# flysoaryun/LF-VIO

Measured on AMD Instinct MI355X. Metric: sliding-window solves/sec (10 KF x N landmarks), higher is better.
Workload: dtype f64; 1 GPU; window300; landmarks=300, observations=1419, windows_per_gpu=1, marginalization=MARGIN_OLD, parallelism=1 independent window stream(s), one per GPU, no data-path collective

## Files before the change

lf-vio_amd/csrc/kernels_marg.h:

```cpp
#pragma once
#include "kernels_solve.h"

constexpr int MARG_THREADS = 768;
constexpr int MARG_MAXD = 96;
constexpr int LDN = 80;
constexpr double JACOBI_TOL = 1e-19;
constexpr size_t MARG_LDS = (size_t)19072 * sizeof(double);
constexpr int BT_GROUP = 4;

DEV void gauge_landmarks(Slot *S, int l0) {
  const int l = l0 + (int)threadIdx.x;
  double *lam = S->lam[S->tr.cur];
  if (l < S->N) lam[l] = 1.0 / (1.0 / lam[l]);
}
template <class T>
DEV void copy_rounds(T *dst, const T *src, int n, int tid, int nthr) {
  for (int k0 = tid; k0 < n; k0 += 8 * nthr) {
    T v[8];
#pragma unroll
    for (int q = 0; q < 8; q++) v[q] = src[k0 + q * nthr < n ? k0 + q * nthr : 0];
#pragma unroll
    for (int q = 0; q < 8; q++)
      if (k0 + q * nthr < n) dst[k0 + q * nthr] = v[q];
  }
}
DEV void gauge_poses(Slot *S, int gated, bool publish);
DEV void publish_solution(Slot *S) {
  char *m = (char *)S->mail;
  if (!m) return;
  const int tid = threadIdx.x, nthr = blockDim.x;
  const TRState *ts = &S->tr;
  const int cur = ts->cur, N = S->N;
  {
    constexpr int XW = (int)(sizeof(FrameState) / 8), XT = (XW + 63) / 64, LT = (SPEC_MAX_LM + 63) / 64, TT = 8;
    const double *xs = (const double *)&S->x[cur];
    double *xd = (double *)(m + MAIL_X + (size_t)cur * sizeof(FrameState));
    const long long *tsrc = (const long long *)ts;
    long long *tdst = (long long *)(m + MAIL_TR);
    const int tl = ts->trace_len < LFVIO_MAX_TRACE ? ts->trace_len : LFVIO_MAX_TRACE;
    const int words = (int)((offsetof(TRState, trace) + (size_t)(tl > 0 ? tl : 0) * sizeof(LfvioIterationSummary)) / 8);
    const double *ls = S->lam[cur];
    double *ld = (double *)(m + MAIL_LAM + (size_t)cur * MAIL_LAM_STRIDE);
    if (nthr >= 64 && XW <= XT * nthr && N <= LT * nthr && words <= TT * nthr) {
      double xv[XT], lv[LT];
      long long tv[TT];
#pragma unroll
      for (int k = 0; k < XT; k++) xv[k] = xs[tid + nthr * k < XW ? tid + nthr * k : 0];
#pragma unroll
      for (int k = 0; k < LT; k++) lv[k] = ls[tid + nthr * k < N ? tid + nthr * k : 0];
#pragma unroll
      for (int k = 0; k < TT; k++) tv[k] = tsrc[tid + nthr * k < words ? tid + nthr * k : 0];
#pragma unroll
      for (int k = 0; k < XT; k++)
        if (tid + nthr * k < XW) xd[tid + nthr * k] = xv[k];
#pragma unroll
      for (int k = 0; k < TT; k++)
        if (tid + nthr * k < words) tdst[tid + nthr * k] = tv[k];
#pragma unroll
      for (int k = 0; k < LT; k++)
        if (tid + nthr * k < N) ld[tid + nthr * k] = lv[k];
    } else {
      for (int k = tid; k < XW; k += nthr) xd[k] = xs[k];
      for (int k = tid; k < words; k += nthr) tdst[k] = tsrc[k];
      for (int k = tid; k < N; k += nthr) ld[k] = ls[k];
    }
  }
  if (tid == 0) ((int *)m)[4] = S->passes_used, ((int *)m)[5] = S->chain_err;
  __threadfence_system();
  __syncthreads();
  if (tid == 0) __hip_atomic_store((int *)m, S->mail_seq, __ATOMIC_RELEASE, __HIP_MEMORY_SCOPE_SYSTEM);
}
DEV void publish_prior(Slot *S) {
  char *m = (char *)S->mail;
  if (!m) return;
  const int tid = threadIdx.x, nthr = blockDim.x;
  const LfvioPrior *src = &S->prior_out;
  LfvioPrior *dst = (LfvioPrior *)(m + MAIL_PRIOR);
  const int n = src->valid == 1 ? src->n : 0;
  copy_rounds((long long *)dst, (const long long *)src, (int)(offsetof(LfvioPrior, linearized_jacobians) / 8), tid, nthr);
  copy_rounds(dst->linearized_jacobians, src->linearized_jacobians, n * n, tid, nthr);
  copy_rounds(dst->linearized_residuals, src->linearized_residuals, n, tid, nthr);
  if (tid == 0) ((int *)m)[2] = S->passes_used, ((int *)m)[3] = S->tr.iteration;
  __threadfence_system();
  __syncthreads();
  if (tid == 0) __hip_atomic_store((int *)m + 1, S->mail_seq, __ATOMIC_RELEASE, __HIP_MEMORY_SCOPE_SYSTEM);
}
__global__ __launch_bounds__(256) void k_publish(char *base, size_t stride) {
  Slot *S = SLOT(base, stride);
  if (!(S->tr.done && (S->tail_state == 0 || S->tail_state == 3))) return;
  publish_solution(S);
}
__global__ __launch_bounds__(256) void k_prior_chain(char *base, size_t stride) {
  Slot *S = SLOT(base, stride);
  const LfvioPrior *src = &S->prior_out;
  const int tid = threadIdx.x, n = S->prior_n, nb = S->prior_nb;
  __shared__ int late;
  if (tid == 0) {
    late = 0;
    const long long t0 = wall_clock64();
    while (spec_peek(&S->tail_state) == 3) {
      if (wall_clock64() - t0 > 10 * SPEC_WAIT_TICKS) {
        late = 1;
        break;
      }
      __builtin_amdgcn_s_sleep(8);
    }
    spec_acquire();
  }
  __syncthreads();
  __shared__ int differs;
  if (tid == 0) differs = 0;
  __syncthreads();
  const bool head = !late && src->valid == 1 && src->n == n && src->num_blocks == nb;
  if (head && tid < nb && !(src->blocks[tid].kind == S->prior_kind[tid] && src->blocks[tid].frame == S->prior_frame[tid] && src->block_idx[tid] == S->prior_idx[tid]))
    differs = 1;
  for (int i = 256 + tid; head && i < nb; i += 256)
    if (!(src->blocks[i].kind == S->prior_kind[i] && src->blocks[i].frame == S->prior_frame[i] && src->block_idx[i] == S->prior_idx[i])) differs = 1;
  __syncthreads();
  const bool same = head && !differs;
  if (!same) {
    if (tid == 0) S->prior_valid = 0, S->chain_err = 1;
    return;
  }
  double *J = S->prior_J, *r = S->prior_r;
  copy_rounds(J, src->linearized_jacobians, n * n, tid, 256);
  copy_rounds(r, src->linearized_residuals, n, tid, 256);
  copy_rounds(&S->prior_x0[0][0], &src->block_x0[0][0], nb * 9, tid, 256);
}
__global__ __launch_bounds__(128) void k_gauge(char *base, size_t stride, int gated) {
  Slot *S = SLOT(base, stride);
  if (gated && !tail_gate(S, S->tr.done)) return;
  if (blockIdx.x > 0) {
    gauge_landmarks(S, (blockIdx.x - 1) * 128);
    return;
  }
  gauge_poses(S, gated, false);
  if (gated && S->spec_on && threadIdx.x == 0) spec_settle(S);
}
__global__ __launch_bounds__(128) void k_decide_gauge(char *base, size_t stride, int publish) {
  Slot *S = SLOT(base, stride);
  decide_body(S);
  __syncthreads();
  if (!tail_gate(S, S->tr.done)) return;
  const int spec = S->spec_on;
  if (spec) {
    if (threadIdx.x == 0) spec_closing(S);
    __syncthreads();
  }
  {
    constexpr int LT = (SPEC_MAX_LM + 127) / 128;
    double *lam = S->lam[S->tr.cur];
    const int N = S->N, tid = threadIdx.x;
    double lv[LT];
#pragma unroll
    for (int k = 0; k < LT; k++) lv[k] = lam[tid + 128 * k < N ? tid + 128 * k : 0];
#pragma unroll
    for (int k = 0; k < LT; k++)
      if (tid + 128 * k < N) lam[tid + 128 * k] = 1.0 / (1.0 / lv[k]);
    for (int l0 = 128 * LT; l0 < N; l0 += 128) gauge_landmarks(S, l0);
  }
  gauge_poses(S, 1, publish != 0);
  if (spec && threadIdx.x == 0) spec_settle(S);
}
DEV void gauge_poses(Slot *S, int gated, bool publish) {
  TRState *ts = &S->tr;
  const int tid = threadIdx.x;
  __shared__ double rot[9], P0[3], oP0[3];
  FrameState *x = &S->x[ts->cur];
  if (tid == 0) {
    const m33 Rs0 = q2R(q_from_pose(S->x0.pose[0]));
    const m33 R00 = q2R(q_from_pose(x->pose[0]));
    const double h0 = sqrt(Rs0.a[0] * Rs0.a[0] + Rs0.a[3] * Rs0.a[3]), h00 = sqrt(R00.a[0] * R00.a[0] + R00.a[3] * R00.a[3]);
    const double c0 = Rs0.a[0] / h0, s0 = Rs0.a[3] / h0, c00 = R00.a[0] / h00, s00 = R00.a[3] / h00;
    const double cyd = c0 * c00 + s0 * s00, syd = s0 * c00 - c0 * s00;
    m33 rd;
    rd.a[0] = cyd, rd.a[1] = -syd, rd.a[2] = 0;
    rd.a[3] = syd, rd.a[4] = cyd, rd.a[5] = 0;
    rd.a[6] = 0, rd.a[7] = 0, rd.a[8] = 1;
    const double sin1deg = 0.017452406437283512;
    if (h0 < sin1deg || h00 < sin1deg) rd = mm(Rs0, tr(R00));
    for (int k = 0; k < 9; k++) rot[k] = rd.a[k];
    for (int k = 0; k < 3; k++) P0[k] = x->pose[0][k], oP0[k] = S->x0.pose[0][k];
  }
  __syncthreads();
  const m33 rd = ldm(rot);
  d3 Psi = mk3(0, 0, 0), Vsi = Psi;
  q4 qn = q4{1, 0, 0, 0};
  if (tid < 11) {
    const m33 Rsi = mm(rd, q2R(qnormalized(q_from_pose(x->pose[tid]))));
    Psi = mul(rd, ld3(x->pose[tid]) - ld3(P0)) + ld3(oP0);
    Vsi = mul(rd, ld3(x->sb[tid]));
    qn = R2q(Rsi);
  } else if (tid == 11) {
    qn = R2q(q2R(q_from_pose(x->ex)));
  }
  __syncthreads();
  __shared__ double bt[84 + TAB_SCRATCH];
  if (tid < 11) {
    const double pn[7] = {Psi.x, Psi.y, Psi.z, qn.x, qn.y, qn.z, qn.w};
#pragma unroll
    for (int k = 0; k < 7; k++) x->pose[tid][k] = pn[k], bt[7 * tid + k] = pn[k];
    x->sb[tid][0] = Vsi.x, x->sb[tid][1] = Vsi.y, x->sb[tid][2] = Vsi.z;
  } else if (tid == 11) {
    x->ex[3] = qn.x, x->ex[4] = qn.y, x->ex[5] = qn.z, x->ex[6] = qn.w;
#pragma unroll
    for (int k = 0; k < 3; k++) bt[77 + k] = x->ex[k];
    bt[80] = qn.x, bt[81] = qn.y, bt[82] = qn.z, bt[83] = qn.w;
  }
  __syncthreads();
  if (publish) publish_solution(S);
  if (tid == 0) {
    if (!gated) ts->done = 0;
    ts->do_lin = 1;
    ts->do_schur = 1;
    ts->chol_fail = 0;
  }
  build_tab(bt, &S->tab[ts->cur], tid, bt + 84);
}

__global__ __launch_bounds__(64) void k_spec_wait(char *base) {
  Slot *S = (Slot *)base;
  if (threadIdx.x != 0) return;
  const long long t0 = wall_clock64();
  while (spec_peek(&S->tail_state) == 3 && wall_clock64() - t0 < 10 * SPEC_WAIT_TICKS) __builtin_amdgcn_s_sleep(8);
}
__global__ __launch_bounds__(128) void k_spec_begin(char *base, size_t back) {
  Slot *S = (Slot *)base;
  Slot *S0 = (Slot *)(base - back);
  const int tid = threadIdx.x;
  __shared__ int sh_word, sh_go;
  const long long t0 = wall_clock64();
  for (;;) {
    if (tid == 0) {
      int go = 0, w = 0;
      const int last = S->shadow.last_word;
      for (;;) {
        const int f = spec_peek(&S0->spec.fin);
        w = spec_peek(&S0->spec.word);
        if (w != 0) {
          const int st = spec_ep(f) == spec_ep(w) ? spec_fin_state(f) : FIN_OPEN;
          if (st != FIN_OPEN) break;
          if (w != last) {
            go = 1;
            break;
          }
        }
        if (wall_clock64() - t0 > SPEC_WAIT_TICKS) break;
        __builtin_amdgcn_s_sleep(8);
      }
      spec_acquire();
      sh_word = w, sh_go = go;
    }
    __syncthreads();
    int go = __builtin_amdgcn_readfirstlane(sh_go);
    const int w = __builtin_amdgcn_readfirstlane(sh_word);
    if (!go) {
      if (tid == 0) S->shadow.word = 0, S->tr.done = 0;
      return;
    }
    const int ep = spec_ep(w), a = spec_acc(w), cur = w & 1;
    if (S->shadow.hdr_ep != ep) {
      const long long *src = (const long long *)S0;
      long long *dst = (long long *)S;
      constexpr int W0 = (int)(offsetof(Slot, lm_start) / 8), W1 = (int)(offsetof(Slot, x) / 8);
      static_assert(offsetof(Slot, lm_start) % 8 == 0 && offsetof(Slot, x) % 8 == 0, "header words");
      for (int k = tid; k < W1; k += 128) dst[k] = src[k] - (k >= W0 ? (long long)back : 0ll);
      const double *is = &S0->imu_sqrt[0][0];
      double *id = &S->imu_sqrt[0][0];
      for (int k = tid; k < LFVIO_WINDOW_SIZE * 225; k += 128) id[k] = is[k];
    }
    __syncthreads();
    {
      constexpr int XW = (int)(sizeof(FrameState) / 8), TW = (int)(sizeof(TRHead) / 8), XT = (XW + 127) / 128, LT = (SPEC_MAX_LM + 127) / 128;
      static_assert(TW <= 128, "the trust-region header in one trip");
      const double *xs = (const double *)&S0->x[cur];
      double *xd = (double *)&S->x[0];
      const double *ls = S0->lam[cur];
      double *ld = S->lam[0];
      const int N = S0->N;
      const long long *ts = (const long long *)&S0->tr;
      long long *td = (long long *)&S->tr;
      double xv[XT], lv[LT];
#pragma unroll
      for (int k = 0; k < XT; k++) xv[k] = xs[tid + 128 * k < XW ? tid + 128 * k : 0];
#pragma unroll
      for (int k = 0; k < LT; k++) lv[k] = ls[tid + 128 * k < N ? tid + 128 * k : 0];
      const long long tv = ts[tid < TW ? tid : 0];
#pragma unroll
      for (int k = 0; k < XT; k++)
        if (tid + 128 * k < XW) xd[tid + 128 * k] = xv[k];
#pragma unroll
      for (int k = 0; k < LT; k++)
        if (tid + 128 * k < N) ld[tid + 128 * k] = 1.0 / (1.0 / lv[k]);
      if (tid < TW) td[tid] = tv;
      for (int k = tid + 128 * LT; k < N; k += 128) ld[k] = 1.0 / (1.0 / ls[k]);
    }
    __syncthreads();
    if (tid == 0) {
      const int f = spec_ld(&S0->spec.fin), w2 = spec_ld(&S0->spec.word);
      const bool open = spec_ep(f) != ep || spec_fin_state(f) == FIN_OPEN;
      sh_go = (w2 == w && open && spec_cas(&S0->spec.own[a], SPEC_FREE, SPEC_SIDE) == SPEC_FREE) ? 1 : 0;
      S->shadow.hdr_ep = ep;
      S->shadow.last_word = w;
    }
    __syncthreads();
    go = __builtin_amdgcn_readfirstlane(sh_go);
    if (!go) {
      __syncthreads();
      continue;
    }
    if (tid == 0) {
      S->shadow.word = w, S->shadow.ticket = S0->spec.ticket;
      S->spec_on = 0, S->dec_pending = 0, S->tail_state = 0, S->chain_err = 0;
      S->tr.cur = 0, S->tr.done = 1;
    }
    __syncthreads();
    break;
  }
  gauge_poses(S, 1, false);
}

DEV bool spd_inverse_wave(const double *Am, double *Xout, int m, int lane, double floor) {
  double a[15];
#pragma unroll
  for (int j = 0; j < 15; j++) a[j] = (lane < m && j < m) ? Am[lane * m + j] : (lane == j ? 1.0 : 0.0);
  bool ok = true;
  double dinv = 1.0;
#pragma unroll
  for (int j = 0; j < 15; j++) {
    const double d = readlane_f64(a[j], j);
    ok = ok && (d > 0.0);
    const double rs = fast_rsqrt(d);
    const double l = lane == j ? d * rs : a[j] * rs;
    a[j] = l;
    dinv = lane == j ? rs : dinv;
#pragma unroll
    for (int c = j + 1; c < 15; c++) a[c] = fma(-l, readlane_f64(l, c), a[c]);
  }
  double y[15];
#pragma unroll
  for (int i = 0; i < 15; i++) {
    double t = lane == i ? 1.0 : 0.0;
#pragma unroll
    for (int k = 0; k < i; k++) t = fma(-readlane_f64(a[k], i), y[k], t);
    y[i] = t * readlane_f64(dinv, i);
  }
  double fro = 0;
#pragma unroll
  for (int r = 0; r < 15; r++) {
    double x = 0;
#pragma unroll
    for (int i = r; i < 15; i++) x = fma(readlane_f64(y[i], r), y[i], x);
    if (lane < m && r < m) Xout[r * m + lane] = x, fro += x * x;
  }
  fro = wave_sum(fro);
  return ok && fro * floor * floor < 1.0;
}

DEV void rr_pair(int k, int step, int np, int n, int &p, int &q) {
  if (k == 0) {
    p = step, q = np - 1;
  } else {
    p = step + k;
    if (p >= np - 1) p -= np - 1;
    q = step - k;
    if (q < 0) q += np - 1;
  }
  if (q >= n) q = -1;
}

DEV void jacobi_angle(double app, double aqq, double apq, double &c, double &s) {
  c = 1.0, s = 0.0;
  if (apq != 0.0 && fabs(apq) > 1e-18 * (fabs(app) + fabs(aqq))) {
#if defined(JAC_TRIVIAL)
    c = 0.8, s = 0.6;
#elif defined(JAC_IEEE)
    const double theta = (aqq - app) / (2.0 * apq);
    const double t = (theta >= 0 ? 1.0 : -1.0) / (fabs(theta) + sqrt(theta * theta + 1.0));
    c = rsqrt(t * t + 1.0);
    s = t * c;
#else
    const double d = aqq - app, e = 2.0 * apq;
    const double h2 = fma(d, d, e * e);
    const double h = h2 * fast_rsqrt(h2);
    const double t = (d >= 0 ? e : -e) * fast_rcp(fabs(d) + h);
    c = fast_rsqrt(fma(t, t, 1.0));
    s = t * c;
#endif
  }
}

DEV int jacobi_small(double *Am, double *Vm, int n, int tid, int nthreads, double *buf, double2 *cs, double *scratch) {
  const int np = n + (n & 1), half = np / 2;
  double *Ac = buf, *An = buf + 256, *Vc = buf + 512, *Vn = buf + 768;
  const bool act = tid < np * np;
  const int u = act ? tid / np : 0, v = act ? tid % np : 0;
  const int ku = u >> 1, bu = u & 1, kv = v >> 1, bv = v & 1;
  auto idx0 = [&](int p) { return (p & 1) ? np - 1 - (p >> 1) : (p >> 1); };
  auto sigma = [&](int p) {
    const int k = p >> 1;
    if (!(p & 1)) return k >= 1 ? 2 * (k - 1) : 3;
    if (k == 0) return 1;
    return k <= half - 2 ? 2 * (k + 1) + 1 : 2 * (half - 1);
  };
  if (act) {
    const int iu = idx0(u), iv = idx0(v);
    Ac[tid] = (iu < n && iv < n) ? Am[iu * n + iv] : 0.0;
    Vc[tid] = (u == iv) ? 1.0 : 0.0;
  }
  const int dst_a = sigma(u) * np + sigma(v), dst_v = u * np + sigma(v);
  const int blk = (2 * ku) * np + 2 * kv;
  __syncthreads();
  int sweeps = 0, g = 0;
  double prev_off = 1e300;
  for (int sweep = 0; sweep < JMAX_SWEEPS; sweep++) {
    double off = 0, dia = 0;
    if (act) {
      const double a = Ac[tid];
      if (u == v) dia = a * a;
      else off = a * a;
    }
    off = wave_sum(off), dia = wave_sum(dia);
    if ((tid & 63) == 0) scratch[tid >> 6] = off, scratch[16 + (tid >> 6)] = dia;
    __syncthreads();
    double so = 0, sd = 0;
    for (int w = 0; w < nthreads / 64; w++) so += scratch[w], sd += scratch[16 + w];
    __syncthreads();
    if (so <= 1e-24 * sd || so == 0.0) break;
    if (sweep >= 4 && so > 0.25 * prev_off) break;
    prev_off = so;
    sweeps++;
    for (int step = 0; step < np - 1; step++, g++) {
      if (tid < half) {
        const int p = 2 * tid, q = p + 1;
        double c = 1.0, s = 0.0;
        if (tid > 0 || np == n) jacobi_angle(Ac[p * np + p], Ac[q * np + q], Ac[q * np + p], c, s);
        cs[tid] = make_double2(c, s);
      }
      __syncthreads();
      if (act) {
        const double2 ra = cs[ku], rb = cs[kv];
        const double ru0 = bu ? ra.y : ra.x, ru1 = bu ? ra.x : -ra.y;
        const double cv0 = bv ? rb.y : rb.x, cv1 = bv ? rb.x : -rb.y;
        const double a00 = Ac[blk], a01 = Ac[blk + 1], a10 = Ac[blk + np], a11 = Ac[blk + np + 1];
        An[dst_a] = ru0 * fma(a00, cv0, a01 * cv1) + ru1 * fma(a10, cv0, a11 * cv1);
        Vn[dst_v] = fma(Vc[u * np + 2 * kv], cv0, Vc[u * np + 2 * kv + 1] * cv1);
      }
      __syncthreads();
      double *t = Ac;
      Ac = An, An = t, t = Vc, Vc = Vn, Vn = t;
    }
  }
  if (act) {
    int p, q;
    rr_pair(kv, g % (np - 1), np, n, p, q);
    const int iv = bv ? q : p;
    if (u == v && iv >= 0) Am[iv * n + iv] = Ac[tid];
    if (u < n && iv >= 0) Vm[u * n + iv] = Vc[tid];
  }
  __syncthreads();
  return sweeps;
}

typedef const __attribute__((address_space(4))) double sdouble;
#define STURM_TOUCH8(v) asm volatile("" ::"s"(v[0]), "s"(v[1]), "s"(v[2]), "s"(v[3]), "s"(v[4]), "s"(v[5]), "s"(v[6]), "s"(v[7]))
DEV int sturm_count(sdouble *Tg , int n, double sigma) {
  double pm = 1.0, p = Tg[0] - sigma;
  unsigned cnt = (unsigned)__double2hiint(p) >> 31;
  unsigned bits = (unsigned)__double2hiint(p) >> 31;
  double d0[8], e0[8], d1[8], e1[8];
#pragma unroll
  for (int u = 0; u < 8; u++) d0[u] = Tg[1 + u], e0[u] = Tg[96 + u];
  for (int i0 = 1; i0 < n; i0 += 16) {
    STURM_TOUCH8(d0);
    STURM_TOUCH8(e0);
#pragma unroll
    for (int u = 0; u < 8; u++) d1[u] = Tg[i0 + 8 + u], e1[u] = Tg[96 + i0 + 8 + u - 1];
#pragma unroll
    for (int u = 0; u < 8; u++) {
      const double pn = fma(d0[u] - sigma, p, -e0[u] * pm);
      bits = __builtin_amdgcn_alignbit(bits, (unsigned)__double2hiint(pn), 31);
      pm = p, p = pn;
    }
    STURM_TOUCH8(d1);
    STURM_TOUCH8(e1);
#pragma unroll
    for (int u = 0; u < 8; u++) d0[u] = Tg[i0 + 16 + u], e0[u] = Tg[96 + i0 + 16 + u - 1];
#pragma unroll
    for (int u = 0; u < 8; u++) {
      const double pn = fma(d1[u] - sigma, p, -e1[u] * pm);
      bits = __builtin_amdgcn_alignbit(bits, (unsigned)__double2hiint(pn), 31);
      pm = p, p = pn;
    }
    cnt += __builtin_popcount((bits ^ (bits >> 1)) & 0xffffu);
    const int ex = ilogb(fmax(fmax(fabs(p), fabs(pm)), 1e-300));
    p = ldexp(p, -ex), pm = ldexp(pm, -ex);
  }
  return (int)cnt;
}
struct TriCtx {
  double *dd, *ee, *tau, *vb0, *vb1, *pp, *RV;
  int n, r0, c0;
};
template <int P>
DEV void tri_finish_row(const TriCtx &tc, int kk, const double (&row)[5], bool own) {
  const int n = tc.n, c0 = tc.c0;
  double *vb = (kk & 1) ? tc.vb1 : tc.vb0;
  double a_part = 0.0, ss_part = 0.0, dk = 0.0;
  bool has_d = false;
#pragma unroll
  for (int q = P; q < 5; q++) {
    const int C = c0 + 16 * q;
    if (C == kk) dk = row[q], has_d = true;
    if (C == kk + 1) a_part = row[q];
    if (C > kk + 1 && C < n) ss_part = fma(row[q], row[q], ss_part);
  }
  if (own && has_d) tc.dd[kk] = dk;
  if (kk + 2 >= n) {
    if (own && kk == n - 2 && c0 == ((n - 1) & 15)) tc.ee[kk] = a_part;
    return;
  }
  a_part = sum8(a_part), ss_part = sum8(ss_part);
  const double alpha = a_part + dpp_f64<0x140>(a_part), ss = ss_part + dpp_f64<0x140>(ss_part);
  const double nn = fma(alpha, alpha, ss);
  const bool live = ss > 0.0;
  const double rs = fast_rsqrt(live ? nn : 1.0);
  const double beta = live ? -copysign(nn * rs, alpha) : alpha;
  const double t = live ? (beta - alpha) * -copysign(rs, alpha) : 0.0;
  const double scal = live ? fast_rcp(alpha - beta) : 0.0;
  if (own) {
#pragma unroll
    for (int q = P; q < 5; q++) {
      const int C = c0 + 16 * q;
      const double v = C == kk + 1 ? 1.0 : ((C > kk + 1 && C < n) ? row[q] * scal : 0.0);
      vb[C] = v;
      if (C > kk && C < n) tc.RV[kk * 76 + C - kk - 1] = v;
    }
    if (c0 == 0) tc.tau[kk] = t, tc.ee[kk] = beta;
  }
}
template <int P>
DEV void tri_matvec(const TriCtx &tc, int k, const double (&ar)[5][5], double (&vj)[5]) {
  const double *vb = (k & 1) ? tc.vb1 : tc.vb0;
  const double t = tc.tau[k];
#pragma unroll
  for (int q = P; q < 5; q++) vj[q] = vb[tc.c0 + 16 * q];
  double sacc[5];
#pragma unroll
  for (int i = P; i < 5; i++) {
    sacc[i] = 0.0;
#pragma unroll
    for (int q = P; q < 5; q++) sacc[i] = fma(ar[i][q], vj[q], sacc[i]);
  }
#pragma unroll
  for (int i = P; i < 5; i++) sacc[i] += dpp_f64<0xB1>(sacc[i]);
#pragma unroll
  for (int i = P; i < 5; i++) sacc[i] += dpp_f64<0x4E>(sacc[i]);
#pragma unroll
  for (int i = P; i < 5; i++) sacc[i] += dpp_f64<0x141>(sacc[i]);
#pragma unroll
  for (int i = P; i < 5; i++) sacc[i] += dpp_f64<0x140>(sacc[i]);
  if (tc.c0 == 0) {
#pragma unroll
    for (int i = P; i < 5; i++) tc.pp[tc.r0 + 16 * i] = tc.r0 + 16 * i > k ? t * sacc[i] : 0.0;
  }
}
template <int P>
DEV void tri_update(const TriCtx &tc, int k, double (&ar)[5][5], const double (&vj)[5]) {
  const double *vb = (k & 1) ? tc.vb1 : tc.vb0;
  const double t = tc.tau[k];
  double pj[5], vi[5], pi[5], pvs = 0.0;
#pragma unroll
  for (int q = P; q < 5; q++) pj[q] = tc.pp[tc.c0 + 16 * q];
#pragma unroll
  for (int i = P; i < 5; i++) vi[i] = vb[tc.r0 + 16 * i], pi[i] = tc.pp[tc.r0 + 16 * i];
#pragma unroll
  for (int q = P; q < 5; q++) pvs = fma(pj[q], vj[q], pvs);
  pvs = sum8(pvs);
  pvs += dpp_f64<0x140>(pvs);
  const double K2 = t * pvs;
#pragma unroll
  for (int i = P; i < 5; i++) {
#pragma unroll
    for (int q = P; q < 5; q++) ar[i][q] = fma(-pi[i], vj[q], fma(-vi[i], pj[q], ar[i][q]));
  }
#pragma unroll
  for (int i = P; i < 5; i++) {
    const double kv = K2 * vi[i];
#pragma unroll
    for (int q = P; q < 5; q++) ar[i][q] = fma(kv, vj[q], ar[i][q]);
    if (i == P) tri_finish_row<P>(tc, k + 1, ar[P], tc.r0 == ((k + 1) & 15));
  }
}
template <int QM, int NR>
DEV void bt_apply(const double *RV, const double *tau, int k, int n, int l8, double (&zz)[10]) {
  double vq[NR][10], tk[NR];
#pragma unroll
  for (int r = 0; r < NR; r++) {
    const int kr = k - r;
    const double *v = RV + kr * 76 - (kr + 1);
    tk[r] = tau[kr];
#pragma unroll
    for (int q = QM; q < 10; q++) {
      const int i = l8 + 8 * q;
      if (QM == 0) vq[r][q] = (i > kr && i < n) ? v[i] : 0.0;
      else vq[r][q] = (q > QM || i > kr) ? v[i] : 0.0;
    }
  }
#pragma unroll
  for (int r = 0; r < NR; r++) {
    double s0 = 0.0, s1 = 0.0;
#pragma unroll
    for (int q = QM; q < 10; q++) {
      if ((q - QM) & 1) s1 = fma(vq[r][q], zz[q], s1);
      else s0 = fma(vq[r][q], zz[q], s0);
    }
    const double s = sum8(s0 + s1) * tk[r];
#pragma unroll
    for (int q = QM; q < 10; q++) zz[q] = fma(-s, vq[r][q], zz[q]);
  }
}
template <int NR>
DEV void bt_dispatch(const double *RV, const double *tau, int k, int n, int l8, double (&zz)[10]) {
  switch (k >> 3) {
    case 0: bt_apply<0, NR>(RV, tau, k, n, l8, zz); break;
    case 1: bt_apply<1, NR>(RV, tau, k, n, l8, zz); break;
    case 2: bt_apply<2, NR>(RV, tau, k, n, l8, zz); break;
    case 3: bt_apply<3, NR>(RV, tau, k, n, l8, zz); break;
    case 4: bt_apply<4, NR>(RV, tau, k, n, l8, zz); break;
    case 5: bt_apply<5, NR>(RV, tau, k, n, l8, zz); break;
    case 6: bt_apply<6, NR>(RV, tau, k, n, l8, zz); break;
    case 7: bt_apply<7, NR>(RV, tau, k, n, l8, zz); break;
    case 8: bt_apply<8, NR>(RV, tau, k, n, l8, zz); break;
    default: bt_apply<9, NR>(RV, tau, k, n, l8, zz); break;
  }
}
DEV double guard_pivot(double q, double pivmin) { return copysign(fmax(fabs(q), pivmin), q); }
template <bool SPEC>
DEV bool eig_tridiag(double *A, const double *b, int n, int tid, double *RV, double *DM, double *vec, double *scr, double *nn2, double *Tglob, LfvioPrior *out, double eps, long long *dbg,
                     SpecPoll *sp_) {
  SpecPoll *const sp = SPEC ? sp_ : nullptr;
  const bool poller = SPEC && tid == MARG_THREADS - 1;
#define ESTAMP(k) do { if (tid == 0) dbg[k] = (long long)__builtin_readcyclecounter(); } while (0)
  ESTAMP(26);
  const int wave = tid >> 6, lane = tid & 63;
  double *dd = vec, *ee = vec + 96, *ee2 = vec + 192, *tau = vec + 288, *lam = vec + 384, *pp = vec + 480, *nrm = vec + 576;
  const bool tri = tid < 256;
  const int r0 = (tid >> 4) & 15, c0 = tid & 15;
  double ar[5][5];
#pragma unroll
  for (int i = 0; i < 5; i++)
#pragma unroll
    for (int q = 0; q < 5; q++) {
      const int R = r0 + 16 * i, C = c0 + 16 * q;
      ar[i][q] = (tri && R < n && C < n) ? A[max(R, C) * LDN + min(R, C)] : 0.0;
    }
  double *vb0 = lam, *vb1 = nrm;
  if (tid < 96) dd[tid] = 0.0, ee[tid] = 0.0, ee2[tid] = 0.0, tau[tid] = 0.0, vb0[tid] = 0.0, vb1[tid] = 0.0;
  for (int e = tid; e < 76 * 76; e += MARG_THREADS) RV[e] = 0.0;
  __syncthreads();
  TriCtx tc = {dd, ee, tau, vb0, vb1, pp, RV, n, r0, c0};
  if (tri) tri_finish_row<0>(tc, 0, ar[0], r0 == 0);
  __syncthreads();
  for (int k = 0; k + 2 < n; k++) {
    const int P = (k + 1) >> 4;
    double vj[5];
    if (poller) {
      if ((k & 7) == 0) spec_poll_issue(*sp);
      else if ((k & 7) == 6) spec_poll_take(*sp);
    }
#ifdef LFVIO_TRI_PROFILE
#define TSTAMP(j) do { if (tid == 0 && k == LFVIO_TRI_PROFILE) dbg[3 + j] = (long long)__builtin_readcyclecounter(); } while (0)
#else
#define TSTAMP(j) do { } while (0)
#endif
    TSTAMP(0);
    if (tri) {
      switch (P) {
        case 0: tri_matvec<0>(tc, k, ar, vj); break;
        case 1: tri_matvec<1>(tc, k, ar, vj); break;
        case 2: tri_matvec<2>(tc, k, ar, vj); break;
        case 3: tri_matvec<3>(tc, k, ar, vj); break;
        default: tri_matvec<4>(tc, k, ar, vj); break;
      }
    }
    TSTAMP(1);
    __syncthreads();
    TSTAMP(2);
    if (tri) {
      switch (P) {
        case 0: tri_update<0>(tc, k, ar, vj); break;
        case 1: tri_update<1>(tc, k, ar, vj); break;
        case 2: tri_update<2>(tc, k, ar, vj); break;
        case 3: tri_update<3>(tc, k, ar, vj); break;
        default: tri_update<4>(tc, k, ar, vj); break;
      }
    }
    TSTAMP(3);
    __syncthreads();
    TSTAMP(4);
    if (sp && (k & 7) == 6 && *sp->flag) return true;
  }
  if (tri) {
#pragma unroll
    for (int i = 0; i < 5; i++)
#pragma unroll
      for (int q = 0; q < 5; q++)
        if (r0 + 16 * i == n - 1 && c0 + 16 * q == n - 1) dd[n - 1] = ar[i][q];
  }
  if (poller) spec_poll_issue(*sp);
  __syncthreads();
  ESTAMP(27);
  if (tid < n) ee2[tid] = ee[tid] * ee[tid];
  {
    double lo = 1e300, hi = -1e300;
    if (tid < n) {
      const double r = (tid > 0 ? fabs(ee[tid - 1]) : 0.0) + (tid + 1 < n ? fabs(ee[tid]) : 0.0);
      lo = dd[tid] - r, hi = dd[tid] + r;
    }
    lo = -wave_max(-lo), hi = wave_max(hi);
    if (lane == 0) scr[wave] = lo, scr[16 + wave] = hi;
  }
  __syncthreads();
  double gl = fmin(scr[0], scr[1]), gu = fmax(scr[16], scr[17]);
  {
    const double tn = fmax(fabs(gl), fabs(gu));
    gl -= 2.2e-16 * tn * n + 1e-300, gu += 2.2e-16 * tn * n + 1e-300;
  }
  if (tid < 96) Tglob[tid] = tid < n ? dd[tid] : gu + 1.0, Tglob[96 + tid] = tid + 1 < n ? ee[tid] * ee[tid] : 0.0;
  __threadfence();
  __syncthreads();
  __builtin_amdgcn_s_dcache_inv();
  const unsigned long long ta = (unsigned long long)Tglob;
  unsigned tlo = __builtin_amdgcn_readfirstlane((unsigned)ta), thi = __builtin_amdgcn_readfirstlane((unsigned)(ta >> 32));
  asm volatile("" : "+s"(tlo), "+s"(thi));
  sdouble *Tg = (sdouble *)(((unsigned long long)thi << 32) | tlo);
  {
    const double pivmin = 1e-290;
    const int g3 = lane == 63 ? 20 : lane / 3, l8 = lane == 63 ? 3 : lane - 3 * g3;
    const int m = wave * 21 + g3;
    const int mm = m < n ? m : n - 1;
    {
      int *cntg = (int *)pp;
      double *blo = nn2, *bhi = nn2 + 96;
      const double step = (gu - gl) * (1.0 / 257.0);
      if (tid < 96) blo[tid] = gl, bhi[tid] = gu;
      if (tid < 256) cntg[tid] = sturm_count(Tg, n, gl + step * (double)(tid + 1));
      __syncthreads();
      if (tid <= 256) {
        const int c0 = tid > 0 ? cntg[tid - 1] : 0, c1 = tid < 256 ? cntg[tid] : n;
        const double a = tid > 0 ? gl + step * (double)tid : gl, b = tid < 256 ? gl + step * (double)(tid + 1) : gu;
        for (int e = max(c0, 0); e < min(c1, n); e++) blo[e] = a, bhi[e] = b;
      }
      __syncthreads();
    }
    double lo = nn2[mm], hi = nn2[96 + mm];
    if (tid < 256)
      for (int round = 0; round < 23; round++) {
        const double w = hi - lo;
        const double sigma = lo + w * (double)(l8 < 3 ? l8 + 1 : 1) * 0.25;
        const int cnt = sturm_count(Tg, n, sigma);
        const int f1 = cnt <= mm ? 1 : 0;
        const unsigned long long bal = __ballot(f1);
        const int f = __builtin_popcount((unsigned)(bal >> (3 * g3)) & 7u);
        const double nlo = f == 0 ? lo : lo + w * (double)f * 0.25, nhi = f == 3 ? hi : lo + w * (double)(f + 1) * 0.25;
        lo = nlo, hi = nhi;
      }
    if (tid < 256 && m < n && l8 == 0) lam[m] = 0.5 * (lo + hi);
    if (poller) spec_poll_take(*sp), spec_poll_issue(*sp);
    __syncthreads();
    ESTAMP(28);
    if (sp && *sp->flag) return true;
    const int set = tid >> 7, me = tid & 127;
    const bool work = set < 2 && me < n;
    const int mec = work ? me : 0;
    const double l = lam[mec];
    if (work && set == 0) {
      double q = dd[0] - l;
      A[mec] = q;
      for (int i0 = 1; i0 < n; i0 += 8) {
        double dv[8], ev[8], qs[8];
#pragma unroll
        for (int u = 0; u < 8; u++) dv[u] = dd[i0 + u], ev[u] = ee2[i0 + u - 1];
#pragma unroll
        for (int u = 0; u < 8; u++) {
          q = fma(-ev[u], fast_rcp(guard_pivot(q, pivmin)), dv[u] - l);
          qs[u] = q;
        }
#pragma unroll
        for (int u = 0; u < 8; u++)
          if (i0 + u < n) A[(i0 + u) * LDN + mec] = qs[u];
      }
    } else if (work) {
      double q = dd[n - 1] - l;
      DM[(n - 1) * LDN + mec] = q;
      for (int i0 = n - 2; i0 >= 0; i0 -= 8) {
        double dv[8], ev[8], qs[8];
#pragma unroll
        for (int u = 0; u < 8; u++) dv[u] = dd[max(i0 - u, 0)], ev[u] = ee2[max(i0 - u, 0)];
#pragma unroll
        for (int u = 0; u < 8; u++) {
          q = fma(-ev[u], fast_rcp(guard_pivot(q, pivmin)), dv[u] - l);
          qs[u] = q;
        }
#pragma unroll
        for (int u = 0; u < 8; u++)
          if (i0 - u >= 0) DM[(i0 - u) * LDN + mec] = qs[u];
      }
    }
    __syncthreads();
    ESTAMP(16);
    {
      const int half = (n + 1) >> 1, i0 = set == 0 ? 0 : half, i1 = set == 0 ? half : n;
      double gmin = 1e300;
      int kt = i0;
      if (work) {
#pragma unroll 8
        for (int i = i0; i < i1; i++) {
          const double g = fabs(A[i * LDN + mec] + DM[i * LDN + mec] - (dd[i] - l));
          if (g < gmin) gmin = g, kt = i;
        }
      }
      __syncthreads();
      if (work) {
        pp[set * 96 + mec] = gmin;
        ((int *)ee2)[set * 96 + mec] = kt;
      }
    }
    if (poller) spec_poll_take(*sp);
    __syncthreads();
    ESTAMP(17);
    if (sp && *sp->flag) return true;
    if (work) {
      const double g0 = pp[mec], g1 = pp[96 + mec];
      const int kt = g1 < g0 ? ((int *)ee2)[96 + mec] : ((int *)ee2)[mec];
      double z = 1.0, nn = 0.0;
      if (set == 0) {
        A[kt * LDN + mec] = 1.0;
        for (int i0 = n - 2; i0 >= 0; i0 -= 8) {
          double c[8], zs[8];
#pragma unroll
          for (int u = 0; u < 8; u++) {
            const int i = max(i0 - u, 0);
            c[u] = -ee[i] * fast_rcp(guard_pivot(A[i * LDN + mec], pivmin));
          }
#pragma unroll
          for (int u = 0; u < 8; u++) {
            const bool on = i0 - u < kt && i0 - u >= 0;
            z = on ? c[u] * z : 1.0;
            zs[u] = z;
            nn = on ? fma(z, z, nn) : nn;
          }
#pragma unroll
          for (int u = 0; u < 8; u++)
            if (i0 - u < kt && i0 - u >= 0) A[(i0 - u) * LDN + mec] = zs[u];
        }
      } else {
        for (int i0 = 1; i0 < n; i0 += 8) {
          double c[8], zs[8];
#pragma unroll
          for (int u = 0; u < 8; u++) {
            const int i = min(i0 + u, n - 1);
            c[u] = -ee[i - 1] * fast_rcp(guard_pivot(DM[i * LDN + mec], pivmin));
          }
#pragma unroll
          for (int u = 0; u < 8; u++) {
            const bool on = i0 + u > kt && i0 + u < n;
            z = on ? c[u] * z : 1.0;
            zs[u] = z;
            nn = on ? fma(z, z, nn) : nn;
          }
#pragma unroll
          for (int u = 0; u < 8; u++)
            if (i0 + u > kt && i0 + u < n) A[(i0 + u) * LDN + mec] = zs[u];
        }
      }
      nn2[set * 96 + mec] = nn;
    }
  }
  __syncthreads();
  ESTAMP(29);
  {
    const int m = tid >> 3, l8 = tid & 7;
    const bool live = m < n;
    const int mm = live ? m : 0;
    double zz[10];
    const double sc = fast_rsqrt(1.0 + nn2[mm] + nn2[96 + mm]);
#pragma unroll
    for (int q = 0; q < 10; q++) {
      const int i = l8 + 8 * q;
      zz[q] = i < n ? A[i * LDN + mm] * sc : 0.0;
    }
    int k = n - 3;
    for (; k >= 0 && (k & (BT_GROUP - 1)) != BT_GROUP - 1; k--) bt_dispatch<1>(RV, tau, k, n, l8, zz);
    for (; k >= 0; k -= BT_GROUP) bt_dispatch<BT_GROUP>(RV, tau, k, n, l8, zz);
    const double l = lam[mm];
    double rb = 0.0;
#pragma unroll
    for (int q = 0; q < 10; q++) {
      const int i = l8 + 8 * q;
      if (i < n) rb = fma(zz[q], b[i], rb);
    }
    rb = sum8(rb);
    if (live) {
      const bool keep = l > eps;
      const double sq = keep ? sqrt(l) : 0.0;
#pragma unroll
      for (int q = 0; q < 10; q++) {
        const int i = l8 + 8 * q;
        if (i < n) out->linearized_jacobians[m * n + i] = sq * zz[q];
      }
      if (l8 == 0) out->linearized_residuals[m] = keep ? rb / sq : 0.0;
    }
  }
  return false;
}

DEV void spec_deliver(Slot *S, Slot *S0, int my_word, bool publish) {
  const int tid = threadIdx.x, nthr = blockDim.x;
  __shared__ int give;
  if (tid == 0) {
    const int ep = spec_ep(my_word), a = spec_acc(my_word);
    long long t0 = wall_clock64();
    int g = 0;
    for (;;) {
      const int f = spec_peek(&S0->spec.fin), w = spec_peek(&S0->spec.word);
      if (spec_ep(w) != ep) break;
      const int st = spec_ep(f) == ep ? spec_fin_state(f) : FIN_OPEN;
      if (st >= FIN_MAIN) {
        g = st == FIN_SIDE && spec_fin_acc(f) == a;
        break;
      }
      if (w != my_word) break;
      if (wall_clock64() - t0 > SPEC_WAIT_TICKS) {
        if (spec_cas(&S0->spec.own[a], SPEC_SIDE, SPEC_ABANDON) == SPEC_SIDE) break;
        t0 = wall_clock64();
      }
      __builtin_amdgcn_s_sleep(8);
    }
    give = g;
  }
  __syncthreads();
  if (!give) return;
  const LfvioPrior *src = &S->prior_out;
  LfvioPrior *dst = &S0->prior_out;
  const int n = src->valid == 1 ? src->n : 0;
  copy_rounds((long long *)dst, (const long long *)src, (int)(offsetof(LfvioPrior, linearized_jacobians) / 8), tid, nthr);
  copy_rounds(dst->linearized_jacobians, src->linearized_jacobians, n * n, tid, nthr);
  copy_rounds(dst->linearized_residuals, src->linearized_residuals, n, tid, nthr);
  __syncthreads();
  if (publish) publish_prior(S0);
  char *m = (char *)S0->mail;
  if (tid == 0) {
    __threadfence_system();
    __hip_atomic_store(&S0->tail_state, 2, __ATOMIC_RELAXED, __HIP_MEMORY_SCOPE_AGENT);
    if (m) __hip_atomic_store((int *)m + 7, S->shadow.ticket, __ATOMIC_RELAXED, __HIP_MEMORY_SCOPE_SYSTEM);
  }
}

template <bool WORKER>
__global__ __launch_bounds__(MARG_THREADS) void k_marg_solve(char *base, size_t stride, int flag_bits) {
  extern __shared__ __attribute__((aligned(16))) double smem[];
  const int flag = flag_bits & 255, force_eig = (flag_bits >> 8) & 1, gated = (flag_bits >> 9) & 1;
  const int publish = (flag_bits >> 10) & 1;
  constexpr bool worker = WORKER;
  Slot *S = worker ? (Slot *)base : SLOT(base, stride);
  Slot *S0 = worker ? (Slot *)(base - stride) : S;
  __shared__ int spec_flag;
  SpecPoll sp{S0, worker ? S->shadow.word : 0, &spec_flag, 0, 0};
  if (threadIdx.x == 0) spec_flag = 0;
  const bool poller = worker && threadIdx.x == MARG_THREADS - 1;
  TRState *tr = &S->tr;
  const MargPlan *mp = &S->marg[flag];
  const int tid = threadIdx.x;
  LfvioPrior *out = &S->prior_out;
  if (gated && !tail_gate(S, tr->done)) return;
  if (worker && sp.my_word == 0) return;
  if (!mp->valid) {
    if (tid == 0) out->valid = -1;
    if (worker) {
      __syncthreads();
      spec_deliver(S, S0, sp.my_word, publish != 0);
      return;
    }
    if (gated && tid == 0) S->iters_done = tr->iteration, S->tail_state = 2;
    if (gated && publish) {
      __syncthreads();
      publish_prior(S);
    }
    return;
  }
  if (poller) spec_poll_issue(sp);
  STAMP(S, 10);
  const double *Sc = S->schur_sum;
  const bool sub = mp->N0 > 0 || S->sharded;
  const int m15 = mp->m15, n = mp->n, D = m15 + n;
  double *Ag = S->mscr;
  double *A = smem;
  double *bv = A + 92 * 92;
  double *Am = bv + 96;
  double *Vm = Am + 256;
  double *Ainv = Vm + 256;
  double *Tm = Ainv + 256;
  double *Ar = smem + 12544;
  double *br = Ar + 76 * LDN;
  double2 *cs = (double2 *)(br + 80);
  int *perm = (int *)(cs + 96);
  double *scr = (double *)(perm + 96);
  double *RV = smem, *vec8 = smem + 5776, *DMs = smem + 5776 + 672;
  for (int c = tid; c < KP; c += MARG_THREADS) {
    const int a = mp->col[c];
    if (a >= 0) perm[a] = c;
  }
  __syncthreads();
  {
    constexpr int GR = (92 * 92 + MARG_THREADS - 1) / MARG_THREADS;
    const double *Hp = &S->Hpp[0];
    double hv[GR], sv[GR];
#pragma unroll
    for (int k = 0; k < GR; k++) {
      const int e = tid + MARG_THREADS * k, ec = e < D * D ? e : 0;
      const int r = D ? perm[ec / max(D, 1)] : 0, c = D ? perm[ec % max(D, 1)] : 0;
      const int hi = max(r, c), lo = min(r, c);
      hv[k] = Hp[hi * (hi + 1) / 2 + lo];
      sv[k] = (sub && hi < KC) ? Sc[schur_index(lo, hi)] : 0.0;
    }
#pragma unroll
    for (int k = 0; k < GR; k++) {
      const int e = tid + MARG_THREADS * k;
      if (e < D * D) A[e] = hv[k] - sv[k];
    }
  }
  for (int a = tid; a < D; a += MARG_THREADS) {
    const int c = perm[a];
    double v = S->gp[c];
    if (sub && c < KC) v -= Sc[schur_index(c, COL_B)];
    bv[a] = v;
  }
  if (poller) spec_poll_take(sp), spec_poll_issue(sp);
  __syncthreads();
  STAMP(S, 11);
  if (worker && spec_flag) return;
  for (int e = tid; e < m15 * m15; e += MARG_THREADS) {
    const int r = e / m15, c = e % m15;
    Am[e] = 0.5 * (A[r * D + c] + A[c * D + r]);
  }
  __syncthreads();
  const double eps = 1e-8;
  __shared__ int spd_fast;
  if (tid < 64) {
    const bool fast = m15 <= 15 && !force_eig && spd_inverse_wave(Am, Ainv, m15, tid, 1e3 * eps);
    if (tid == 0) spd_fast = fast ? 1 : 0;
  }
  __syncthreads();
  int sw1 = 0;
  if (!spd_fast) {
    sw1 = jacobi_small(Am, Vm, m15, tid, MARG_THREADS, Tm, cs, scr);
    __syncthreads();
    for (int e = tid; e < m15 * m15; e += MARG_THREADS) {
      const int r = e / m15, c = e % m15;
      double s = 0;
      for (int k = 0; k < m15; k++) {
        const double ev = Am[k * m15 + k];
        if (ev > eps) s += Vm[r * m15 + k] * (1.0 / ev) * Vm[c * m15 + k];
      }
      Ainv[e] = s;
    }
    __syncthreads();
  }
  STAMP(S, 12);
  for (int e = tid; e < n * m15; e += MARG_THREADS) {
    const int r = e / m15, c = e % m15;
    double s = 0;
    for (int k = 0; k < m15; k++) s = fma(A[(m15 + r) * D + k], Ainv[k * m15 + c], s);
    Tm[e] = s;
  }
  __syncthreads();
  {
    const int nb4 = (n + 3) >> 2;
    for (int blk = tid; blk < nb4 * nb4; blk += MARG_THREADS) {
      const int r0 = 4 * (blk / nb4), c0 = 4 * (blk % nb4);
      double acc[4][4];
#pragma unroll
      for (int i = 0; i < 4; i++)
#pragma unroll
        for (int j = 0; j < 4; j++) acc[i][j] = 0.0;
      for (int k = 0; k < m15; k++) {
        double tv[4], av[4];
#pragma unroll
        for (int i = 0; i < 4; i++) tv[i] = Tm[min(r0 + i, n - 1) * m15 + k], av[i] = A[k * D + m15 + min(c0 + i, n - 1)];
#pragma unroll
        for (int i = 0; i < 4; i++)
#pragma unroll
          for (int j = 0; j < 4; j++) acc[i][j] = fma(tv[i], av[j], acc[i][j]);
      }
#pragma unroll
      for (int i = 0; i < 4; i++)
#pragma unroll
        for (int j = 0; j < 4; j++)
          if (r0 + i < n && c0 + j < n) Ar[(r0 + i) * LDN + c0 + j] = A[(m15 + r0 + i) * D + m15 + c0 + j] - acc[i][j];
    }
  }
  for (int r = tid; r < n; r += MARG_THREADS) {
    double s = 0;
    for (int k = 0; k < m15; k++) s = fma(Tm[r * m15 + k], bv[k], s);
    br[r] = bv[m15 + r] - s;
  }
  __syncthreads();
  double *Aout = Ag + 92 * 92 + 96;
  for (int e = tid; e < n * n; e += MARG_THREADS) {
    const int r = e / n, c = e % n;
    Aout[e] = Ar[max(r, c) * LDN + min(r, c)];
  }
  for (int r = tid; r < n; r += MARG_THREADS) Aout[n * n + r] = br[r];
  if (poller) spec_poll_take(sp);
  __syncthreads();
  if (worker && spec_flag) return;
  STAMP(S, 13);
  if (eig_tridiag<WORKER>(Ar, br, n, tid, RV, DMs, vec8, scr, (double *)cs, S->eig_aux, out, 1e-8, S->dbg, &sp)) return;
  if (tid == 0) S->dbg[24] = sw1;
  STAMP(S, 14);
  const FrameState *x = &S->x[tr->cur];
  if (tid < mp->nb) {
    const int kind = mp->kind[tid], frame = mp->frame[tid];
    out->blocks[tid].kind = kind;
    out->blocks[tid].frame = mp->shifted_frame[tid];
    out->block_idx[tid] = mp->idx[tid];
    const double *xb = kind == LFVIO_BLOCK_POSE ? x->pose[frame]
                       : kind == LFVIO_BLOCK_SPEEDBIAS ? x->sb[frame]
                       : kind == LFVIO_BLOCK_EX_POSE ? x->ex
                                                     : &x->td;
    const int gs = (kind == LFVIO_BLOCK_POSE || kind == LFVIO_BLOCK_EX_POSE) ? 7 : (kind == LFVIO_BLOCK_SPEEDBIAS ? 9 : 1);
    for (int k = 0; k < 9; k++) out->block_x0[tid][k] = k < gs ? xb[k] : 0.0;
  }
  STAMP(S, 15);
  if (tid == 0) {
    out->valid = 1;
    out->m = m15 + (S->sharded ? (int)(S->xch[XOFF_C + XS_N0] + 0.5) : mp->N0);
    out->n = n;
    out->num_blocks = mp->nb;
    if (gated && !worker) S->iters_done = tr->iteration, S->tail_state = 2;
  }
  if (worker) {
    __syncthreads();
    spec_deliver(S, S0, sp.my_word, publish != 0);
    return;
  }
  if (gated && publish) {
    __syncthreads();
    publish_prior(S);
  }
}
```

Before: 2413 solves/s.

## Keep Householder vectors in registers and drop one barrier per tridiagonalization step

Each thread now carries the current Householder column vector and tau in registers. The row view of the vector is obtained with a ds_bpermute lane shuffle, where before it was read from shared-memory vb buffers. The next pivot row is staged in a double-buffered rb array and updated separately, so the next reflector is computed before the full trailing update. This allows the second __syncthreads per step to be removed and the first to be replaced with a lighter lds_barrier. The aim is to cut barrier and LDS round-trip latency in the serial tridiagonalization loop, at the cost of more register pressure and subtle correctness risk from the reduced synchronization.

```diff
diff --git a/lf-vio_amd/csrc/kernels_marg.h b/lf-vio_amd/csrc/kernels_marg.h
--- a/lf-vio_amd/csrc/kernels_marg.h
+++ b/lf-vio_amd/csrc/kernels_marg.h
@@ -499,21 +499,23 @@
   return (int)cnt;
 }
 struct TriCtx {
-  double *dd, *ee, *tau, *vb0, *vb1, *pp, *RV;
+  double *dd, *ee, *tau, *pp, *rb, *RV;
   int n, r0, c0;
 };
+struct TriRefl {
+  double vj[5], vi[5], tau;
+};
 template <int P>
-DEV void tri_finish_row(const TriCtx &tc, int kk, const double (&row)[5], bool own) {
+DEV void tri_finish_row(const TriCtx &tc, int kk, const double (&rowc)[5], bool own, double (&nvj)[5], double &ntau) {
   const int n = tc.n, c0 = tc.c0;
-  double *vb = (kk & 1) ? tc.vb1 : tc.vb0;
   double a_part = 0.0, ss_part = 0.0, dk = 0.0;
   bool has_d = false;
 #pragma unroll
   for (int q = P; q < 5; q++) {
     const int C = c0 + 16 * q;
-    if (C == kk) dk = row[q], has_d = true;
-    if (C == kk + 1) a_part = row[q];
-    if (C > kk + 1 && C < n) ss_part = fma(row[q], row[q], ss_part);
+    if (C == kk) dk = rowc[q], has_d = true;
+    if (C == kk + 1) a_part = rowc[q];
+    if (C > kk + 1 && C < n) ss_part = fma(rowc[q], rowc[q], ss_part);
   }
   if (own && has_d) tc.dd[kk] = dk;
   if (kk + 2 >= n) {
@@ -528,29 +530,38 @@
   const double beta = live ? -copysign(nn * rs, alpha) : alpha;
   const double t = live ? (beta - alpha) * -copysign(rs, alpha) : 0.0;
   const double scal = live ? fast_rcp(alpha - beta) : 0.0;
+#pragma unroll
+  for (int q = P; q < 5; q++) {
+    const int C = c0 + 16 * q;
+    nvj[q] = C == kk + 1 ? 1.0 : ((C > kk + 1 && C < n) ? rowc[q] * scal : 0.0);
+  }
+  ntau = t;
   if (own) {
 #pragma unroll
     for (int q = P; q < 5; q++) {
       const int C = c0 + 16 * q;
-      const double v = C == kk + 1 ? 1.0 : ((C > kk + 1 && C < n) ? row[q] * scal : 0.0);
-      vb[C] = v;
-      if (C > kk && C < n) tc.RV[kk * 76 + C - kk - 1] = v;
+      if (C > kk && C < n) tc.RV[kk * 76 + C - kk - 1] = nvj[q];
     }
     if (c0 == 0) tc.tau[kk] = t, tc.ee[kk] = beta;
   }
 }
 template <int P>
-DEV void tri_matvec(const TriCtx &tc, int k, const double (&ar)[5][5], double (&vj)[5]) {
-  const double *vb = (k & 1) ? tc.vb1 : tc.vb0;
-  const double t = tc.tau[k];
-#pragma unroll
-  for (int q = P; q < 5; q++) vj[q] = vb[tc.c0 + 16 * q];
+DEV void tri_rows_from_columns(const TriCtx &tc, TriRefl &rf) {
+  const int src = (((int)threadIdx.x & 48) | tc.r0) << 2;
+#pragma unroll
+  for (int i = P; i < 5; i++)
+    rf.vi[i] = __hiloint2double(__builtin_amdgcn_ds_bpermute(src, __double2hiint(rf.vj[i])), __builtin_amdgcn_ds_bpermute(src, __double2loint(rf.vj[i])));
+}
+template <int P>
+DEV void tri_matvec(const TriCtx &tc, int k, const double (&ar)[5][5], const TriRefl &rf) {
+  double *pp = tc.pp + 96 * (k & 1), *rb = tc.rb + 96 * (k & 1);
+  const double t = rf.tau;
   double sacc[5];
 #pragma unroll
   for (int i = P; i < 5; i++) {
     sacc[i] = 0.0;
 #pragma unroll
-    for (int q = P; q < 5; q++) sacc[i] = fma(ar[i][q], vj[q], sacc[i]);
+    for (int q = P; q < 5; q++) sacc[i] = fma(ar[i][q], rf.vj[q], sacc[i]);
   }
 #pragma unroll
   for (int i = P; i < 5; i++) sacc[i] += dpp_f64<0xB1>(sacc[i]);
@@ -560,37 +571,52 @@
   for (int i = P; i < 5; i++) sacc[i] += dpp_f64<0x141>(sacc[i]);
 #pragma unroll
   for (int i = P; i < 5; i++) sacc[i] += dpp_f64<0x140>(sacc[i]);
+  if (tc.r0 == ((k + 1) & 15)) {
+#pragma unroll
+    for (int q = P; q < 5; q++) rb[tc.c0 + 16 * q] = ar[P][q];
+  }
   if (tc.c0 == 0) {
 #pragma unroll
-    for (int i = P; i < 5; i++) tc.pp[tc.r0 + 16 * i] = tc.r0 + 16 * i > k ? t * sacc[i] : 0.0;
+    for (int i = P; i < 5; i++) pp[tc.r0 + 16 * i] = tc.r0 + 16 * i > k ? t * sacc[i] : 0.0;
   }
 }
 template <int P>
-DEV void tri_update(const TriCtx &tc, int k, double (&ar)[5][5], const double (&vj)[5]) {
-  const double *vb = (k & 1) ? tc.vb1 : tc.vb0;
-  const double t = tc.tau[k];
-  double pj[5], vi[5], pi[5], pvs = 0.0;
-#pragma unroll
-  for (int q = P; q < 5; q++) pj[q] = tc.pp[tc.c0 + 16 * q];
-#pragma unroll
-  for (int i = P; i < 5; i++) vi[i] = vb[tc.r0 + 16 * i], pi[i] = tc.pp[tc.r0 + 16 * i];
-#pragma unroll
-  for (int q = P; q < 5; q++) pvs = fma(pj[q], vj[q], pvs);
+DEV void tri_update(const TriCtx &tc, int k, double (&ar)[5][5], TriRefl &rf) {
+  const double *pp = tc.pp + 96 * (k & 1), *rb = tc.rb + 96 * (k & 1);
+  const double t = rf.tau;
+  double pj[5], pi[5], rowc[5], pvs = 0.0;
+#pragma unroll
+  for (int q = P; q < 5; q++) pj[q] = pp[tc.c0 + 16 * q], rowc[q] = rb[tc.c0 + 16 * q];
+#pragma unroll
+  for (int i = P; i < 5; i++) pi[i] = pp[tc.r0 + 16 * i];
+  const double pk = pp[k + 1], vk = 1.0;
+#pragma unroll
+  for (int q = P; q < 5; q++) pvs = fma(pj[q], rf.vj[q], pvs);
   pvs = sum8(pvs);
   pvs += dpp_f64<0x140>(pvs);
   const double K2 = t * pvs;
+  const double kvk = K2 * vk;
+#pragma unroll
+  for (int q = P; q < 5; q++) rowc[q] = fma(kvk, rf.vj[q], fma(-pk, rf.vj[q], fma(-vk, pj[q], rowc[q])));
+  double nvj[5], ntau = 0.0;
+#pragma unroll
+  for (int q = 0; q < 5; q++) nvj[q] = 0.0;
+  tri_finish_row<P>(tc, k + 1, rowc, tc.r0 == ((k + 1) & 15), nvj, ntau);
 #pragma unroll
   for (int i = P; i < 5; i++) {
 #pragma unroll
-    for (int q = P; q < 5; q++) ar[i][q] = fma(-pi[i], vj[q], fma(-vi[i], pj[q], ar[i][q]));
+    for (int q = P; q < 5; q++) ar[i][q] = fma(-pi[i], rf.vj[q], fma(-rf.vi[i], pj[q], ar[i][q]));
   }
 #pragma unroll
   for (int i = P; i < 5; i++) {
-    const double kv = K2 * vi[i];
-#pragma unroll
-    for (int q = P; q < 5; q++) ar[i][q] = fma(kv, vj[q], ar[i][q]);
-    if (i == P) tri_finish_row<P>(tc, k + 1, ar[P], tc.r0 == ((k + 1) & 15));
-  }
+    const double kv = K2 * rf.vi[i];
+#pragma unroll
+    for (int q = P; q < 5; q++) ar[i][q] = fma(kv, rf.vj[q], ar[i][q]);
+  }
+#pragma unroll
+  for (int q = P; q < 5; q++) rf.vj[q] = nvj[q];
+  rf.tau = ntau;
+  tri_rows_from_columns<P>(tc, rf);
 }
 template <int QM, int NR>
 DEV void bt_apply(const double *RV, const double *tau, int k, int n, int l8, double (&zz)[10]) {
@@ -655,16 +681,26 @@
       const int R = r0 + 16 * i, C = c0 + 16 * q;
       ar[i][q] = (tri && R < n && C < n) ? A[max(R, C) * LDN + min(R, C)] : 0.0;
     }
-  double *vb0 = lam, *vb1 = nrm;
-  if (tid < 96) dd[tid] = 0.0, ee[tid] = 0.0, ee2[tid] = 0.0, tau[tid] = 0.0, vb0[tid] = 0.0, vb1[tid] = 0.0;
+  TriRefl rf;
+  double row0c[5];
+#pragma unroll
+  for (int q = 0; q < 5; q++) {
+    const int C = c0 + 16 * q;
+    row0c[q] = (tri && C < n) ? A[C * LDN] : 0.0;
+    rf.vj[q] = 0.0, rf.vi[q] = 0.0;
+  }
+  rf.tau = 0.0;
+  double *rb = nn2;
+  if (tid < 96) dd[tid] = 0.0, ee[tid] = 0.0, ee2[tid] = 0.0, tau[tid] = 0.0, lam[tid] = 0.0, nrm[tid] = 0.0;
   for (int e = tid; e < 76 * 76; e += MARG_THREADS) RV[e] = 0.0;
   __syncthreads();
-  TriCtx tc = {dd, ee, tau, vb0, vb1, pp, RV, n, r0, c0};
-  if (tri) tri_finish_row<0>(tc, 0, ar[0], r0 == 0);
-  __syncthreads();
+  TriCtx tc = {dd, ee, tau, pp, rb, RV, n, r0, c0};
+  if (tri) {
+    tri_finish_row<0>(tc, 0, row0c, r0 == 0, rf.vj, rf.tau);
+    tri_rows_from_columns<0>(tc, rf);
+  }
   for (int k = 0; k + 2 < n; k++) {
     const int P = (k + 1) >> 4;
-    double vj[5];
     if (poller) {
       if ((k & 7) == 0) spec_poll_issue(*sp);
       else if ((k & 7) == 6) spec_poll_take(*sp);
@@ -677,27 +713,26 @@
     TSTAMP(0);
     if (tri) {
       switch (P) {
-        case 0: tri_matvec<0>(tc, k, ar, vj); break;
-        case 1: tri_matvec<1>(tc, k, ar, vj); break;
-        case 2: tri_matvec<2>(tc, k, ar, vj); break;
-        case 3: tri_matvec<3>(tc, k, ar, vj); break;
-        default: tri_matvec<4>(tc, k, ar, vj); break;
+        case 0: tri_matvec<0>(tc, k, ar, rf); break;
+        case 1: tri_matvec<1>(tc, k, ar, rf); break;
+        case 2: tri_matvec<2>(tc, k, ar, rf); break;
+        case 3: tri_matvec<3>(tc, k, ar, rf); break;
+        default: tri_matvec<4>(tc, k, ar, rf); break;
       }
     }
     TSTAMP(1);
-    __syncthreads();
+    lds_barrier();
     TSTAMP(2);
     if (tri) {
       switch (P) {
-        case 0: tri_update<0>(tc, k, ar, vj); break;
-        case 1: tri_update<1>(tc, k, ar, vj); break;
-        case 2: tri_update<2>(tc, k, ar, vj); break;
-        case 3: tri_update<3>(tc, k, ar, vj); break;
-        default: tri_update<4>(tc, k, ar, vj); break;
+        case 0: tri_update<0>(tc, k, ar, rf); break;
+        case 1: tri_update<1>(tc, k, ar, rf); break;
+        case 2: tri_update<2>(tc, k, ar, rf); break;
+        case 3: tri_update<3>(tc, k, ar, rf); break;
+        default: tri_update<4>(tc, k, ar, rf); break;
       }
     }
     TSTAMP(3);
-    __syncthreads();
     TSTAMP(4);
     if (sp && (k & 7) == 6 && *sp->flag) return true;
   }
```

After: 2394 solves/s. Within noise of the previous version (-0.8%).
